# Gustavroot/DeflatedMLMC_Schwinger

Measured on AMD Instinct MI355X. Metric: hutchinson_probe_samples_per_sec_schwinger128, higher is better.
Workload: dtype f64

## Files before the change

### deflatedmlmc_schwinger_amd/csrc/sw_kernels.hpp

```cpp
#pragma once
#include <hip/hip_runtime.h>
#include <stdint.h>

namespace swk {

typedef double2 cplx;

#define SW_WAVE 64
#define SW_BLOCK 256
#define SW_WAVES_PER_BLOCK 4
#define SW_SHIFT_SMALL_L 256
#define SW_SHIFT_MID_L 768
#define SW_SHIFT_MAX_L 1024

__device__ __forceinline__ cplx cmake(double a, double b) { cplx r; r.x = a; r.y = b; return r; }
__device__ __forceinline__ cplx cadd(cplx a, cplx b) { return cmake(a.x + b.x, a.y + b.y); }
__device__ __forceinline__ cplx csub(cplx a, cplx b) { return cmake(a.x - b.x, a.y - b.y); }
__device__ __forceinline__ cplx cmul(cplx a, cplx b) {
  return cmake(fma(a.x, b.x, -a.y * b.y), fma(a.x, b.y, a.y * b.x));
}
__device__ __forceinline__ cplx cmulc(cplx a, cplx b) {
  return cmake(fma(a.x, b.x, a.y * b.y), fma(a.x, b.y, -a.y * b.x));
}
__device__ __forceinline__ void cfma(cplx& acc, cplx a, cplx b) {
// ... 585 lines not shown
  const int wave = threadIdx.x >> 6;
  const int lane = threadIdx.x & 63;
  const int bx = xcd_remap(blockIdx.x, gridDim.x);
  const int slot = __builtin_amdgcn_readfirstlane(bx * SW_WAVES_PER_BLOCK + wave);
  if (slot >= ngroups) return;
  const int grp = order ? __builtin_amdgcn_readfirstlane(order[slot]) : slot;
  const size_t col = (size_t)blockIdx.y * 64 + lane;
  const int* c = cols + (size_t)grp * K;
  const C* v = vals + (size_t)grp * K * G;
  C acc[G];
#pragma unroll
  for (int g = 0; g < G; ++g) acc[g] = czero<C>();
  const C* Xc = X + col;
  constexpr int UC = (G <= 8) ? 8 : 4;
  int k = 0;
  for (; k + UC <= K; k += UC) {
    C xs[UC];
#pragma unroll
    for (int u = 0; u < UC; ++u) xs[u] = Xc[(size_t)c[k + u] * nbp];
    __builtin_amdgcn_sched_barrier(0);
#pragma unroll
    for (int u = 0; u < UC; ++u) {
#pragma unroll
      for (int g = 0; g < G; ++g) cfma(acc[g], v[(size_t)(k + u) * G + g], xs[u]);
    }
  }
  for (; k < K; ++k) {
    const C x = Xc[(size_t)c[k] * nbp];
#pragma unroll
    for (int g = 0; g < G; ++g) cfma(acc[g], v[(size_t)k * G + g], x);
  }
#pragma unroll
  for (int g = 0; g < G; ++g) {
    const size_t row = (size_t)grp * G + g;
    C o = acc[g];
    if (MODE == 1) o = csub(B[row * nbp + col], o);
    if (MODE == 2) o = cadd(B[row * nbp + col], o);
    if (MODE == 3) {
      C t = X[row * nbp + col];
      cfma(t, w, csub(B[row * nbp + col], o));
      o = t;
    }
    Y[row * nbp + col] = o;
  }
}

typedef double sw_double4 __attribute__((ext_vector_type(4)));
#ifndef SW_BSR_WAVES_NT4
#define SW_BSR_WAVES_NT4 3
#endif
#define SW_BSR_MIN_WAVES(NT_, STG_) (((NT_) == 4 && (STG_) <= 4) ? SW_BSR_WAVES_NT4 : 1)

template <int MODE, int NT, bool NTIO>
__device__ __forceinline__ void bsr_store(const sw_double4 (&re)[NT], const sw_double4 (&im)[NT], int rt,
                                          int c0, int lane, const int* __restrict__ tmap,
                                          const double* __restrict__ Xr,
                                          const double* __restrict__ Br, double* __restrict__ Yr,
                                          int ld, cplx w, const double (*xown)[NT] = nullptr) {
  const int c = lane & 15;
  const bool odd = (c & 1) != 0;
  const int ot = tmap ? __builtin_amdgcn_readfirstlane(tmap[rt]) : rt;
#pragma unroll
  for (int r = 0; r < 4; ++r) {
    const size_t row = (size_t)ot * 16 + (lane >> 4) + 4 * r;
#pragma unroll
    for (int t = 0; t < NT; ++t) {
      const double s = __shfl_xor(im[t][r], 1);
      double y = odd ? re[t][r] + s : re[t][r] - s;
      const size_t off = row * ld + c0 + t * 16 + c;
      if (MODE == 1) y = (NTIO ? __builtin_nontemporal_load(&Br[off]) : Br[off]) - y;
      if (MODE == 3) {
        const double tt = (NTIO ? __builtin_nontemporal_load(&Br[off]) : Br[off]) - y;
        const double tp = __shfl_xor(tt, 1);
        y = (xown ? xown[r][t] : Xr[off]) + w.x * tt + (odd ? w.y * tp : -w.y * tp);
      }
      if (NTIO) __builtin_nontemporal_store(y, &Yr[off]);
      else Yr[off] = y;
    }
  }
}

template <int MODE, int NT, bool NTIO = false, int STG = 2>
__global__ __launch_bounds__(SW_BLOCK, SW_BSR_MIN_WAVES(NT, STG)) void k_bsr_mfma(const cplx* __restrict__ Ap,
                                                       const int* __restrict__ kcol, int KS,
                                                       int RT, const double* __restrict__ Xr,
                                                       const double* __restrict__ Br,
                                                       double* __restrict__ Yr, int ld, int nbp,
                                                       cplx w, int map, int msub,
                                                       const int* __restrict__ tmap, int xreg) {
  const int lane = threadIdx.x & 63;
  const int RB = (RT + SW_WAVES_PER_BLOCK - 1) / SW_WAVES_PER_BLOCK;
  const int NC = (gridDim.y > 1) ? gridDim.y : gridDim.x / RB;
  int bx, cy;
  if (gridDim.y > 1) {
    cy = blockIdx.y;
    bx = xcd_remap(blockIdx.x, RB);
  } else if (map == 0 || map == 3 || (RB & 7)) {
    cy = blockIdx.x / RB;
    bx = xcd_remap(blockIdx.x - cy * RB, RB);
  } else {
    const int xcd = blockIdx.x & 7, j = blockIdx.x >> 3, RBx = RB >> 3;
    if (map == 1 || (RBx % msub)) {
      cy = j % NC;
      bx = xcd * RBx + j / NC;
    } else {
      const int per = NC * msub;
      const int sidx = j / per, rem = j - sidx * per;
      cy = rem / msub;
      bx = xcd * RBx + sidx * msub + (rem - cy * msub);
    }
  }
  const int rt = __builtin_amdgcn_readfirstlane(bx * SW_WAVES_PER_BLOCK + (threadIdx.x >> 6));
  if (rt >= RT) return;
  const int c0 = cy * (16 * NT);
  const cplx* a = Ap + (size_t)rt * KS * 64 + lane;
  const int* kc = kcol + (size_t)rt * KS;
  const double* b = Xr + (size_t)(lane >> 4) * ld + c0 + (lane & 15);
  sw_double4 re[NT], im[NT];
#pragma unroll
  for (int t = 0; t < NT; ++t) {
    re[t] = sw_double4{0.0, 0.0, 0.0, 0.0};
    im[t] = re[t];
  }
#define SW_BSR_LOAD(M_, X_, KSI)                               \
  {                                                            \
    M_ = a[(size_t)(KSI) * 64];                                \
    const double* bk_ = b + (size_t)kc[(KSI)] * ld;            \
    _Pragma("unroll") for (int t = 0; t < NT; ++t) X_[t] = bk_[t * 16]; \
  }
#define SW_BSR_MFMA(M_, X_)                                                        \
  _Pragma("unroll") for (int t = 0; t < NT; ++t) {                                 \
    re[t] = __builtin_amdgcn_mfma_f64_16x16x4f64(M_.x, X_[t], re[t], 0, 0, 0);     \
    im[t] = __builtin_amdgcn_mfma_f64_16x16x4f64(M_.y, X_[t], im[t], 0, 0, 0);     \
  }
  cplx mm[STG];
  double xx[STG][NT];
#pragma unroll
  for (int s = 0; s < STG; ++s) SW_BSR_LOAD(mm[s], xx[s], s);
  for (int ks = 0; ks < KS; ks += STG) {
#pragma unroll
    for (int s = 0; s < STG; ++s) {
      const int kn = (ks + s + STG < KS) ? ks + s + STG : ks + s;
      __builtin_amdgcn_sched_barrier(0);
      SW_BSR_MFMA(mm[s], xx[s]);
      __builtin_amdgcn_sched_barrier(0);
      SW_BSR_LOAD(mm[s], xx[s], kn);
    }
  }
#undef SW_BSR_LOAD
#undef SW_BSR_MFMA
  if (MODE == 3 && STG == 4 && xreg) bsr_store<MODE, NT, NTIO>(re, im, rt, c0, lane, tmap, Xr, Br, Yr, ld, w, xx);
  else bsr_store<MODE, NT, NTIO>(re, im, rt, c0, lane, tmap, Xr, Br, Yr, ld, w);
}

#define SW_BSR3_MIN_WAVES(NT_, STG_) (((NT_) <= 2 && (STG_) <= 4) ? 2 : 1)

template <int MODE, int NT, bool NTIO = false, int STG = 4>
__global__ __launch_bounds__(SW_BLOCK, SW_BSR3_MIN_WAVES(NT, STG)) void k_bsr_mfma3(
    const cplx* __restrict__ Ap, const int* __restrict__ kcol, int KS, int RT, const cplx* __restrict__ X,
    const cplx* __restrict__ B, cplx* __restrict__ Y, int nbp, cplx w, int map, int msub,
    const int* __restrict__ tmap, int xreg) {
  const int lane = threadIdx.x & 63;
  const int RB = (RT + SW_WAVES_PER_BLOCK - 1) / SW_WAVES_PER_BLOCK;
  const int NC = gridDim.x / RB;
  int bx, cy;
  if (map == 0 || map == 3 || (RB & 7)) {
    cy = blockIdx.x / RB;
    bx = xcd_remap(blockIdx.x - cy * RB, RB);
  } else {
    const int xcd = blockIdx.x & 7, j = blockIdx.x >> 3, RBx = RB >> 3;
    if (map == 1 || (RBx % msub)) {
      cy = j % NC;
      bx = xcd * RBx + j / NC;
    } else {
      const int per = NC * msub;
      const int sidx = j / per, rem = j - sidx * per;
      cy = rem / msub;
      bx = xcd * RBx + sidx * msub + (rem - cy * msub);
    }
  }
  const int rt = __builtin_amdgcn_readfirstlane(bx * SW_WAVES_PER_BLOCK + (threadIdx.x >> 6));
  if (rt >= RT) return;
  const int c0 = cy * (16 * NT);
  const cplx* a = Ap + (size_t)rt * KS * 64 + lane;
  const int* kc = kcol + (size_t)rt * KS;
  const cplx* b = X + (size_t)(lane >> 4) * nbp + c0 + (lane & 15);
  sw_double4 t1[NT], t2[NT], t3[NT];
#pragma unroll
  for (int t = 0; t < NT; ++t) {
    t1[t] = sw_double4{0.0, 0.0, 0.0, 0.0};
    t2[t] = t1[t];
    t3[t] = t1[t];
  }
#define SW_B3_LOAD(M_, X_, KSI)                                 \
  {                                                             \
    M_ = a[(size_t)(KSI) * 64];                                 \
    const cplx* bk_ = b + (size_t)kc[(KSI)] * nbp;              \
    _Pragma("unroll") for (int t = 0; t < NT; ++t) X_[t] = bk_[t * 16]; \
  }
#define SW_B3_MFMA(M_, X_)                                                                  \
  {                                                                                         \
    const double ms_ = M_.x + M_.y;                                                         \
    _Pragma("unroll") for (int t = 0; t < NT; ++t) {                                        \
      t1[t] = __builtin_amdgcn_mfma_f64_16x16x4f64(M_.x, X_[t].x, t1[t], 0, 0, 0);          \
      t2[t] = __builtin_amdgcn_mfma_f64_16x16x4f64(M_.y, X_[t].y, t2[t], 0, 0, 0);          \
      t3[t] = __builtin_amdgcn_mfma_f64_16x16x4f64(ms_, X_[t].x + X_[t].y, t3[t], 0, 0, 0); \
    }                                                                                       \
  }
  cplx mm[STG];
  cplx xx[STG][NT];
#pragma unroll
  for (int s = 0; s < STG; ++s) SW_B3_LOAD(mm[s], xx[s], (s < KS ? s : 0));
  for (int ks = 0; ks < KS; ks += STG) {
#pragma unroll
    for (int s = 0; s < STG; ++s) {
      if (ks + s < KS) {
        const int kn = (ks + s + STG < KS) ? ks + s + STG : ks + s;
        __builtin_amdgcn_sched_barrier(0);
        SW_B3_MFMA(mm[s], xx[s]);
        __builtin_amdgcn_sched_barrier(0);
        SW_B3_LOAD(mm[s], xx[s], kn);
      }
    }
  }
#undef SW_B3_LOAD
#undef SW_B3_MFMA
  const int ot = tmap ? __builtin_amdgcn_readfirstlane(tmap[rt]) : rt;
  const bool own = MODE == 3 && STG == 4 && xreg && (KS % 4 == 0);
#pragma unroll
  for (int r = 0; r < 4; ++r) {
    const size_t row = (size_t)ot * 16 + (lane >> 4) + 4 * r;
#pragma unroll
    for (int t = 0; t < NT; ++t) {
      const size_t off = row * nbp + c0 + t * 16 + (lane & 15);
      cplx y = cmake(t1[t][r] - t2[t][r], t3[t][r] - t1[t][r] - t2[t][r]);
      if (MODE == 1 || MODE == 3) {
        cplx q;
        if (NTIO) {
          const double* bp_ = (const double*)&B[off];
          q = cmake(__builtin_nontemporal_load(bp_), __builtin_nontemporal_load(bp_ + 1));
        } else {
          q = B[off];
        }
        y = csub(q, y);
      }
      if (MODE == 3) {
        cplx o;
        if constexpr (STG == 4) o = own ? xx[r][t] : X[off];
        else o = X[off];
        cfma(o, w, y);
        y = o;
      }
      if (NTIO) {
        double* yp_ = (double*)&Y[off];
        __builtin_nontemporal_store(y.x, yp_);
        __builtin_nontemporal_store(y.y, yp_ + 1);
      } else {
        Y[off] = y;
      }
    }
  }
}

#define SW_DL_DEPTH 4

template <int RTW, int KB>
__global__ __launch_bounds__(128 * RTW) void k_dense_mfma3_lds(const cplx* __restrict__ Ap,
                                                              const int* __restrict__ kcol, int KS, int RT,
                                                              const cplx* __restrict__ X, cplx* __restrict__ Y,
                                                              int nbp, const int* __restrict__ tmap) {
  constexpr int WAVES = 2 * RTW;
  constexpr int APIECES = RTW * KB, PIECES = APIECES + 2 * KB, PPW = PIECES / WAVES;
  static_assert(PIECES % WAVES == 0, "pieces must divide over the waves");
  __shared__ cplx lds[2][PIECES * 64];
  const int lane = threadIdx.x & 63;
  const int wave = __builtin_amdgcn_readfirstlane((int)(threadIdx.x >> 6));
  const int RB = RT / RTW, NC = nbp >> 5;
  int rb, pc;
  if ((RB & 7) == 0) {
    const int xcd = blockIdx.x & 7, j = blockIdx.x >> 3, RBx = RB >> 3;
    rb = xcd * RBx + j / NC;
    pc = j % NC;
  } else {
    rb = blockIdx.x / NC;
    pc = blockIdx.x % NC;
  }
  const int rtl = wave >> 1, ptl = wave & 1;
  const int rt0 = rb * RTW;
  const int c0 = pc * 32;
  const int nstages = KS / KB;
  static_assert(APIECES % WAVES == 0 && PPW >= 3 && PPW <= 6, "piece layout");
#define SW_DL_SRC(T)                                                                                     \
  ((WAVES * (T) < APIECES)                                                                               \
       ? Ap + ((size_t)(rt0 + (wave + WAVES * (T)) / KB) * KS + ((wave + WAVES * (T)) % KB)) * 64 + lane \
       : X + (size_t)(2 * ((wave + WAVES * (T) - APIECES) & 1) + (lane >> 5)) * nbp + c0 + (lane & 31))
  const cplx* const src0 = SW_DL_SRC(0);
  const cplx* const src1 = SW_DL_SRC(1);
  const cplx* const src2 = SW_DL_SRC(2);
  const cplx* const src3 = (PPW > 3) ? SW_DL_SRC(3) : src2;
  const cplx* const src4 = (PPW > 4) ? SW_DL_SRC(4) : src2;
  const cplx* const src5 = (PPW > 5) ? SW_DL_SRC(5) : src2;
#undef SW_DL_SRC
#define SW_DL_XK(T) ((wave + WAVES * (T) - APIECES) >> 1)
#define SW_DL_LD1(DST, SRC, T, KS0)                                                                \
  if (WAVES * (T) < APIECES) DST = SRC[(size_t)(KS0) * 64];                                        \
  else DST = SRC[(size_t)kcol[(KS0) + SW_DL_XK(T)] * nbp];
#define SW_DL_LOAD(RING, ST)                                                                       \
  {                                                                                                \
    const int ks0_ = min((ST), nstages - 1) * KB;                                                  \
    SW_DL_LD1(RING##_0, src0, 0, ks0_)                                                             \
    SW_DL_LD1(RING##_1, src1, 1, ks0_)                                                             \
    SW_DL_LD1(RING##_2, src2, 2, ks0_)                                                             \
    if (PPW > 3) { SW_DL_LD1(RING##_3, src3, 3, ks0_) }                                            \
    if (PPW > 4) { SW_DL_LD1(RING##_4, src4, 4, ks0_) }                                            \
    if (PPW > 5) { SW_DL_LD1(RING##_5, src5, 5, ks0_) }                                            \
  }
#define SW_DL_WRITE(RING, BUF)                                                                     \
  {                                                                                                \
    lds[BUF][(wave + WAVES * 0) * 64 + lane] = RING##_0;                                           \
    lds[BUF][(wave + WAVES * 1) * 64 + lane] = RING##_1;                                           \
    lds[BUF][(wave + WAVES * 2) * 64 + lane] = RING##_2;                                           \
    if (PPW > 3) lds[BUF][(wave + WAVES * 3) * 64 + lane] = RING##_3;                              \
    if (PPW > 4) lds[BUF][(wave + WAVES * 4) * 64 + lane] = RING##_4;                              \
    if (PPW > 5) lds[BUF][(wave + WAVES * 5) * 64 + lane] = RING##_5;                              \
  }
#define SW_DL_DECL(RING) \
  cplx RING##_0, RING##_1, RING##_2, RING##_3 = cmake(0.0, 0.0), RING##_4 = RING##_3, RING##_5 = RING##_3;
  SW_DL_DECL(ring0)
  SW_DL_DECL(ring1)
  SW_DL_DECL(ring2)
  SW_DL_DECL(ring3)
#undef SW_DL_DECL
  static_assert(SW_DL_DEPTH == 4, "the ring is written out for four stages");
#define SW_DL_STEP(RING, BUF, ST)                                                                  \
  {                                                                                                \
    SW_DL_WRITE(RING, (BUF) ^ 1);                                                                  \
    __builtin_amdgcn_sched_barrier(0);                                                             \
    SW_DL_LOAD(RING, (ST) + 1 + SW_DL_DEPTH);                                                      \
    __builtin_amdgcn_sched_barrier(0);                                                             \
    const cplx* sl_ = &lds[BUF][0];                                                                \
    _Pragma("unroll") for (int k = 0; k < KB; ++k) {                                               \
      const cplx m_ = sl_[a_off + k * 64];                                                         \
      const cplx xv_ = sl_[x_off + k * 128];                                                       \
      t1 = __builtin_amdgcn_mfma_f64_16x16x4f64(m_.x, xv_.x, t1, 0, 0, 0);                         \
      t2 = __builtin_amdgcn_mfma_f64_16x16x4f64(m_.y, xv_.y, t2, 0, 0, 0);                         \
      t3 = __builtin_amdgcn_mfma_f64_16x16x4f64(m_.x + m_.y, xv_.x + xv_.y, t3, 0, 0, 0);          \
    }                                                                                              \
    __syncthreads();                                                                               \
  }
  SW_DL_LOAD(ring0, 0);
  SW_DL_LOAD(ring1, 1);
  SW_DL_LOAD(ring2, 2);
  SW_DL_LOAD(ring3, 3);
  SW_DL_WRITE(ring0, 0);
  __builtin_amdgcn_sched_barrier(0);
  SW_DL_LOAD(ring0, 4);
  __builtin_amdgcn_sched_barrier(0);
  __syncthreads();
  sw_double4 t1 = {0.0, 0.0, 0.0, 0.0}, t2 = t1, t3 = t1;
  const int a_off = (rtl * KB) * 64 + lane;
  const int x_off = (APIECES + (lane >> 5)) * 64 + ((lane >> 4) & 1) * 32 + ptl * 16 + (lane & 15);
  for (int st = 0; st < nstages; st += 4) {
    SW_DL_STEP(ring1, 0, st);
    SW_DL_STEP(ring2, 1, st + 1);
    SW_DL_STEP(ring3, 0, st + 2);
    SW_DL_STEP(ring0, 1, st + 3);
  }
#undef SW_DL_STEP
#undef SW_DL_LOAD
#undef SW_DL_LD1
#undef SW_DL_XK
#undef SW_DL_WRITE
  const int rt = rt0 + rtl;
  const int ot = tmap ? __builtin_amdgcn_readfirstlane(tmap[rt]) : rt;
#pragma unroll
  for (int r = 0; r < 4; ++r) {
    const size_t row = (size_t)ot * 16 + (lane >> 4) + 4 * r;
    Y[row * nbp + c0 + ptl * 16 + (lane & 15)] = cmake(t1[r] - t2[r], t3[r] - t1[r] - t2[r]);
  }
}

typedef float sw_float4 __attribute__((ext_vector_type(4)));

template <int MODE, int NT, int STG>
__global__ __launch_bounds__(SW_BLOCK) void k_bsr_mfma_f32(const cplxf* __restrict__ Ap,
                                                           const int* __restrict__ kcol, int KS,
                                                           int RT, const cplxf* __restrict__ X,
                                                           const cplxf* __restrict__ B,
                                                           cplxf* __restrict__ Y, int nbp, cplxf w,
                                                           int map, const int* __restrict__ tmap) {
  const int lane = threadIdx.x & 63;
  const int RB = (RT + SW_WAVES_PER_BLOCK - 1) / SW_WAVES_PER_BLOCK;
  const int NC = gridDim.x / RB;
  int bx, cy;
  if (map == 0 || (RB & 7)) {
    cy = blockIdx.x / RB;
    bx = xcd_remap(blockIdx.x - cy * RB, RB);
  } else {
    const int xcd = blockIdx.x & 7, j = blockIdx.x >> 3, RBx = RB >> 3;
    cy = j % NC;
    bx = xcd * RBx + j / NC;
  }
  const int rt = __builtin_amdgcn_readfirstlane(bx * SW_WAVES_PER_BLOCK + (threadIdx.x >> 6));
  if (rt >= RT) return;
  const int c0 = cy * (16 * NT);
  const cplxf* a = Ap + (size_t)rt * KS * 64 + lane;
  const int* kc = kcol + (size_t)rt * KS;
  const cplxf* b = X + (size_t)(lane >> 4) * nbp + c0 + (lane & 15);
  sw_float4 re[NT], im[NT];
#pragma unroll
  for (int t = 0; t < NT; ++t) {
    re[t] = sw_float4{0.f, 0.f, 0.f, 0.f};
    im[t] = re[t];
  }
#define SW_BSRF_LOAD(M_, X_, KSI)                               \
  {                                                             \
    M_ = a[(size_t)(KSI) * 64];                                 \
    const cplxf* bk_ = b + (size_t)kc[(KSI)] * nbp;             \
    _Pragma("unroll") for (int t = 0; t < NT; ++t) X_[t] = bk_[t * 16]; \
  }
#define SW_BSRF_MFMA(M_, X_)                                                              \
  {                                                                                       \
    const float nay_ = -M_.y;                                                             \
    _Pragma("unroll") for (int t = 0; t < NT; ++t) {                                      \
      re[t] = __builtin_amdgcn_mfma_f32_16x16x4f32(M_.x, X_[t].x, re[t], 0, 0, 0);        \
      im[t] = __builtin_amdgcn_mfma_f32_16x16x4f32(M_.x, X_[t].y, im[t], 0, 0, 0);        \
    }                                                                                     \
    _Pragma("unroll") for (int t = 0; t < NT; ++t) {                                      \
      re[t] = __builtin_amdgcn_mfma_f32_16x16x4f32(nay_, X_[t].y, re[t], 0, 0, 0);        \
      im[t] = __builtin_amdgcn_mfma_f32_16x16x4f32(M_.y, X_[t].x, im[t], 0, 0, 0);        \
    }                                                                                     \
  }
  cplxf mm[STG];
  cplxf xx[STG][NT];
#pragma unroll
  for (int s = 0; s < STG; ++s) SW_BSRF_LOAD(mm[s], xx[s], (s < KS ? s : 0));
  for (int ks = 0; ks < KS; ks += STG) {
#pragma unroll
    for (int s = 0; s < STG; ++s) {
      if (ks + s < KS) {
        const int kn = (ks + s + STG < KS) ? ks + s + STG : ks + s;
        __builtin_amdgcn_sched_barrier(0);
        SW_BSRF_MFMA(mm[s], xx[s]);
        __builtin_amdgcn_sched_barrier(0);
        SW_BSRF_LOAD(mm[s], xx[s], kn);
      }
    }
  }
#undef SW_BSRF_LOAD
#undef SW_BSRF_MFMA
  const int ot = tmap ? __builtin_amdgcn_readfirstlane(tmap[rt]) : rt;
#pragma unroll
  for (int r = 0; r < 4; ++r) {
    const size_t row = (size_t)ot * 16 + 4 * (lane >> 4) + r;
#pragma unroll
    for (int t = 0; t < NT; ++t) {
      const size_t off = row * nbp + c0 + t * 16 + (lane & 15);
      cplxf y = cmake(re[t][r], im[t][r]);
      if (MODE == 1) y = csub(B[off], y);
      if (MODE == 3) {
        cplxf o = X[off];
        cfma(o, w, csub(B[off], y));
        y = o;
      }
      Y[off] = y;
    }
  }
}

template <int MODE, int NT>
__global__ __launch_bounds__(SW_BLOCK) void k_bsr_mfma_f32_sk(const cplxf* __restrict__ Ap,
                                                              const int* __restrict__ kcol, int KS,
                                                              int RT, const cplxf* __restrict__ X,
                                                              const cplxf* __restrict__ B,
                                                              cplxf* __restrict__ Y, int nbp, cplxf w,
                                                              const int* __restrict__ tmap) {
  __shared__ float red[3][NT * 8][64];
  const int lane = threadIdx.x & 63;
  const int q = threadIdx.x >> 6;
  const int rt = blockIdx.x % RT;
  const int cy = blockIdx.x / RT;
  const int c0 = cy * (16 * NT);
  const cplxf* a = Ap + (size_t)rt * KS * 64 + lane;
  const int* kc = kcol + (size_t)rt * KS;
  const cplxf* b = X + (size_t)(lane >> 4) * nbp + c0 + (lane & 15);
  sw_float4 re[NT], im[NT];
#pragma unroll
  for (int t = 0; t < NT; ++t) {
    re[t] = sw_float4{0.f, 0.f, 0.f, 0.f};
    im[t] = re[t];
  }
  constexpr int STG = 4;
  cplxf mm[STG];
  cplxf xx[STG][NT];
#define SW_SKF_LOAD(S_, KSI)                                                  \
  {                                                                           \
    const int ks_ = ((KSI) < KS) ? (KSI) : q;                                 \
    mm[S_] = a[(size_t)ks_ * 64];                                             \
    const cplxf* bk_ = b + (size_t)kc[ks_] * nbp;                             \
    _Pragma("unroll") for (int t = 0; t < NT; ++t) xx[S_][t] = bk_[t * 16];   \
  }
#pragma unroll
  for (int s = 0; s < STG; ++s) SW_SKF_LOAD(s, q + 4 * s);
  for (int ks = q; ks < KS; ks += 4 * STG) {
#pragma unroll
    for (int s = 0; s < STG; ++s) {
      if (ks + 4 * s < KS) {
        __builtin_amdgcn_sched_barrier(0);
        const float nay = -mm[s].y;
#pragma unroll
        for (int t = 0; t < NT; ++t) {
          re[t] = __builtin_amdgcn_mfma_f32_16x16x4f32(mm[s].x, xx[s][t].x, re[t], 0, 0, 0);
          im[t] = __builtin_amdgcn_mfma_f32_16x16x4f32(mm[s].x, xx[s][t].y, im[t], 0, 0, 0);
        }
#pragma unroll
        for (int t = 0; t < NT; ++t) {
          re[t] = __builtin_amdgcn_mfma_f32_16x16x4f32(nay, xx[s][t].y, re[t], 0, 0, 0);
          im[t] = __builtin_amdgcn_mfma_f32_16x16x4f32(mm[s].y, xx[s][t].x, im[t], 0, 0, 0);
        }
        __builtin_amdgcn_sched_barrier(0);
        SW_SKF_LOAD(s, ks + 4 * s + 4 * STG);
      }
    }
  }
#undef SW_SKF_LOAD
  if (q > 0) {
#pragma unroll
    for (int t = 0; t < NT; ++t)
#pragma unroll
      for (int r = 0; r < 4; ++r) {
        red[q - 1][t * 8 + r][lane] = re[t][r];
        red[q - 1][t * 8 + 4 + r][lane] = im[t][r];
      }
  }
  __syncthreads();
  if (q != 0) return;
  const int ot = tmap ? __builtin_amdgcn_readfirstlane(tmap[rt]) : rt;
#pragma unroll
  for (int r = 0; r < 4; ++r) {
    const size_t row = (size_t)ot * 16 + 4 * (lane >> 4) + r;
#pragma unroll
    for (int t = 0; t < NT; ++t) {
      const size_t off = row * nbp + c0 + t * 16 + (lane & 15);
      cplxf y = cmake(re[t][r] + red[0][t * 8 + r][lane] + red[1][t * 8 + r][lane] + red[2][t * 8 + r][lane],
                      im[t][r] + red[0][t * 8 + 4 + r][lane] + red[1][t * 8 + 4 + r][lane] +
                          red[2][t * 8 + 4 + r][lane]);
      if (MODE == 1) y = csub(B[off], y);
      if (MODE == 3) {
        cplxf o = X[off];
        cfma(o, w, csub(B[off], y));
        y = o;
      }
      Y[off] = y;
    }
  }
}

template <class CI, class CO>
__global__ __launch_bounds__(SW_BLOCK) void k_cast(const CI* __restrict__ src, CO* __restrict__ dst,
                                                   size_t count) {
  const size_t i = (size_t)blockIdx.x * SW_BLOCK + threadIdx.x;
  if (i >= count) return;
  const CI v = src[i];
  CO o;
  o.x = (typename real_of<CO>::type)v.x;
  o.y = (typename real_of<CO>::type)v.y;
  dst[i] = o;
}

__device__ __forceinline__ int blk_pos_row(int q) { return q & 15; }
__device__ __forceinline__ int blk_pos_col(int q) { return 4 * (q >> 6) + ((q & 63) >> 4); }

__global__ __launch_bounds__(256) void k_block_inverse(const cplx* __restrict__ src,
                                                       const long long* __restrict__ soff,
                                                       cplx* __restrict__ dst,
                                                       const long long* __restrict__ doff,
                                                       int* __restrict__ info) {
  __shared__ cplx a[16][33];
  __shared__ cplx fac[16];
  __shared__ int piv;
  const int q = threadIdx.x;
  const int i = blk_pos_row(q), c = blk_pos_col(q);
  const cplx* s = src + soff[blockIdx.x];
  a[i][c] = s[q];
  a[i][16 + c] = cmake(i == c ? 1.0 : 0.0, 0.0);
  __syncthreads();
  for (int k = 0; k < 16; ++k) {
    if (q == 0) {
      int p = k;
      double best = a[k][k].x * a[k][k].x + a[k][k].y * a[k][k].y;
      for (int r = k + 1; r < 16; ++r) {
        const double m = a[r][k].x * a[r][k].x + a[r][k].y * a[r][k].y;
        if (m > best) {
          best = m;
          p = r;
        }
      }
      piv = p;
      if (best == 0.0) atomicOr(info, 1);
    }
    __syncthreads();
    const int p = piv;
    if (p != k && q < 32) {
      const cplx t = a[k][q];
      a[k][q] = a[p][q];
      a[p][q] = t;
    }
    __syncthreads();
    if (q < 16) fac[q] = a[q][k];
    __syncthreads();
    const cplx pv = fac[k];
    const double d = pv.x * pv.x + pv.y * pv.y;
    const cplx ip = d > 0.0 ? cmake(pv.x / d, -pv.y / d) : cmake(0.0, 0.0);
    if (q < 32) a[k][q] = cmul(a[k][q], ip);
    __syncthreads();
#pragma unroll
    for (int e = 0; e < 2; ++e) {
      const int idx = q + 256 * e;
      const int r = idx >> 5, cc = idx & 31;
      if (r != k) {
        const cplx f = fac[r];
        const cplx t = cmul(f, a[k][cc]);
        a[r][cc] = csub(a[r][cc], t);
      }
    }
    __syncthreads();
  }
  dst[doff[blockIdx.x] + q] = a[i][16 + c];
}

__global__ __launch_bounds__(256) void k_block_products(const int* __restrict__ ptr,
                                                        const long long* __restrict__ aoff,
                                                        const long long* __restrict__ boff,
                                                        const cplx* __restrict__ A,
                                                        const cplx* __restrict__ B,
                                                        const long long* __restrict__ ioff,
                                                        const cplx* __restrict__ init, double sign,
                                                        cplx* __restrict__ out,
                                                        const long long* __restrict__ ooff) {
  __shared__ cplx as[16][17], bs[16][17];
  const int q = threadIdx.x;
  const int i = blk_pos_row(q), c = blk_pos_col(q);
  const int b = blockIdx.x;
  cplx acc = cmake(0.0, 0.0);
  for (int t = ptr[b]; t < ptr[b + 1]; ++t) {
    as[i][c] = A[aoff[t] + q];
    bs[i][c] = B[boff[t] + q];
    __syncthreads();
#pragma unroll
    for (int m = 0; m < 16; ++m) cfma(acc, as[i][m], bs[m][c]);
    __syncthreads();
  }
  cplx o = cmake(sign * acc.x, sign * acc.y);
  if (ioff[b] >= 0) o = cadd(o, init[ioff[b] + q]);
  out[ooff[b] + q] = o;
}

__global__ __launch_bounds__(1024) void k_gj_pivot(const cplx* __restrict__ A, int n, int k,
                                                   int* __restrict__ pivs, cplx* __restrict__ pvinv,
                                                   int* __restrict__ info) {
  __shared__ double bm[1024];
  __shared__ int bi[1024];
  const int t = threadIdx.x;
  double best = -1.0;
  int arg = k;
  for (int r = k + t; r < n; r += 1024) {
    const cplx v = A[(size_t)r * n + k];
    const double m = v.x * v.x + v.y * v.y;
    if (m > best) {
      best = m;
      arg = r;
    }
  }
// ... 2788 lines not shown
```

Before: 35060.

## Software-pipeline LDS reads and MFMAs, prefetch kcol indices a stage early

Restructures the inner f64 MFMA loop of the BSR dot kernel so that LDS operand reads for the next k-step, and the complex-sum adds, are interleaved with the MFMAs of the current step. The last MFMA triple of each stage is deferred into the next stage to overlap with its ring write and global load issue. It also loads the kcol column indices into registers one stage ahead, taking the dependent index load off the X gather path. The cost is more live registers and a more intricate schedule held in place by sched_barriers.

Measured after the change: 35260 (median of 4 runs). No clear change (+0.6%).

```diff
diff --git a/deflatedmlmc_schwinger_amd/csrc/sw_kernels.hpp b/deflatedmlmc_schwinger_amd/csrc/sw_kernels.hpp
--- a/deflatedmlmc_schwinger_amd/csrc/sw_kernels.hpp
+++ b/deflatedmlmc_schwinger_amd/csrc/sw_kernels.hpp
@@ -911,9 +911,18 @@
   const cplx* const src5 = (PPW > 5) ? SW_DL_SRC(5) : src2;
 #undef SW_DL_SRC
 #define SW_DL_XK(T) ((wave + WAVES * (T) - APIECES) >> 1)
+  int kc_0 = 0, kc_1 = 0, kc_2 = 0, kc_3 = 0, kc_4 = 0, kc_5 = 0;
+#define SW_DL_KC1(T, KS0) \
+  if ((T) < PPW && WAVES * (T) >= APIECES) kc_##T = kcol[(KS0) + SW_DL_XK(T)];
+#define SW_DL_KC(ST)                                                                               \
+  {                                                                                                \
+    const int kk0_ = min((ST), nstages - 1) * KB;                                                  \
+    SW_DL_KC1(0, kk0_) SW_DL_KC1(1, kk0_) SW_DL_KC1(2, kk0_)                                       \
+    SW_DL_KC1(3, kk0_) SW_DL_KC1(4, kk0_) SW_DL_KC1(5, kk0_)                                       \
+  }
 #define SW_DL_LD1(DST, SRC, T, KS0)                                                                \
   if (WAVES * (T) < APIECES) DST = SRC[(size_t)(KS0) * 64];                                        \
-  else DST = SRC[(size_t)kcol[(KS0) + SW_DL_XK(T)] * nbp];
+  else DST = SRC[(size_t)kc_##T * nbp];
 #define SW_DL_LOAD(RING, ST)                                                                       \
   {                                                                                                \
     const int ks0_ = min((ST), nstages - 1) * KB;                                                  \
@@ -941,32 +950,68 @@
   SW_DL_DECL(ring3)
 #undef SW_DL_DECL
   static_assert(SW_DL_DEPTH == 4, "the ring is written out for four stages");
+  static_assert(KB % 2 == 0, "the k-steps of a stage alternate between two operand sets");
+#define SW_DL_READ(S, BUF, K)                                                                      \
+  {                                                                                                \
+    m##S = lds[BUF][a_off + (K) * 64];                                                             \
+    x##S = lds[BUF][x_off + (K) * 128];                                                            \
+  }
+#define SW_DL_SUMS(S)                                                                              \
+  {                                                                                                \
+    ms##S = m##S.x + m##S.y;                                                                       \
+    xs##S = x##S.x + x##S.y;                                                                       \
+  }
+#define SW_DL_MFMA(S)                                                                              \
+  {                                                                                                \
+    t1 = __builtin_amdgcn_mfma_f64_16x16x4f64(m##S.x, x##S.x, t1, 0, 0, 0);                        \
+    t2 = __builtin_amdgcn_mfma_f64_16x16x4f64(m##S.y, x##S.y, t2, 0, 0, 0);                        \
+    t3 = __builtin_amdgcn_mfma_f64_16x16x4f64(ms##S, xs##S, t3, 0, 0, 0);                          \
+  }
 #define SW_DL_STEP(RING, BUF, ST)                                                                  \
   {                                                                                                \
+    SW_DL_READ(P, BUF, 0);                                                                         \
+    __builtin_amdgcn_sched_barrier(0);                                                             \
+    SW_DL_MFMA(Q);                                                                                 \
+    __builtin_amdgcn_sched_barrier(0);                                                             \
     SW_DL_WRITE(RING, (BUF) ^ 1);                                                                  \
     __builtin_amdgcn_sched_barrier(0);                                                             \
     SW_DL_LOAD(RING, (ST) + 1 + SW_DL_DEPTH);                                                      \
     __builtin_amdgcn_sched_barrier(0);                                                             \
-    const cplx* sl_ = &lds[BUF][0];                                                                \
-    _Pragma("unroll") for (int k = 0; k < KB; ++k) {                                               \
-      const cplx m_ = sl_[a_off + k * 64];                                                         \
-      const cplx xv_ = sl_[x_off + k * 128];                                                       \
-      t1 = __builtin_amdgcn_mfma_f64_16x16x4f64(m_.x, xv_.x, t1, 0, 0, 0);                         \
-      t2 = __builtin_amdgcn_mfma_f64_16x16x4f64(m_.y, xv_.y, t2, 0, 0, 0);                         \
-      t3 = __builtin_amdgcn_mfma_f64_16x16x4f64(m_.x + m_.y, xv_.x + xv_.y, t3, 0, 0, 0);          \
+    _Pragma("unroll") for (int k = 0; k < KB; k += 2) {                                            \
+      SW_DL_SUMS(P);                                                                               \
+      __builtin_amdgcn_sched_barrier(0);                                                           \
+      SW_DL_READ(Q, BUF, k + 1);                                                                   \
+      if (k == KB - 2) SW_DL_KC((ST) + 2 + SW_DL_DEPTH);                                           \
+      __builtin_amdgcn_sched_barrier(0);                                                           \
+      SW_DL_MFMA(P);                                                                               \
+      SW_DL_SUMS(Q);                                                                               \
+      __builtin_amdgcn_sched_barrier(0);                                                           \
+      if (k + 2 < KB) {                                                                            \
+        SW_DL_READ(P, BUF, k + 2);                                                                 \
+        __builtin_amdgcn_sched_barrier(0);                                                         \
+        SW_DL_MFMA(Q);                                                                             \
+      }                                                                                            \
     }                                                                                              \
     __syncthreads();                                                                               \
   }
+  SW_DL_KC(0);
   SW_DL_LOAD(ring0, 0);
+  SW_DL_KC(1);
   SW_DL_LOAD(ring1, 1);
+  SW_DL_KC(2);
   SW_DL_LOAD(ring2, 2);
+  SW_DL_KC(3);
   SW_DL_LOAD(ring3, 3);
+  SW_DL_KC(4);
   SW_DL_WRITE(ring0, 0);
   __builtin_amdgcn_sched_barrier(0);
   SW_DL_LOAD(ring0, 4);
+  SW_DL_KC(1 + SW_DL_DEPTH);
   __builtin_amdgcn_sched_barrier(0);
   __syncthreads();
   sw_double4 t1 = {0.0, 0.0, 0.0, 0.0}, t2 = t1, t3 = t1;
+  cplx mP, xP, mQ = cmake(0.0, 0.0), xQ = mQ;
+  double msP, xsP, msQ = 0.0, xsQ = 0.0;
   const int a_off = (rtl * KB) * 64 + lane;
   const int x_off = (APIECES + (lane >> 5)) * 64 + ((lane >> 4) & 1) * 32 + ptl * 16 + (lane & 15);
   for (int st = 0; st < nstages; st += 4) {
@@ -975,9 +1020,15 @@
     SW_DL_STEP(ring3, 0, st + 2);
     SW_DL_STEP(ring0, 1, st + 3);
   }
+  SW_DL_MFMA(Q);
 #undef SW_DL_STEP
+#undef SW_DL_READ
+#undef SW_DL_SUMS
+#undef SW_DL_MFMA
 #undef SW_DL_LOAD
 #undef SW_DL_LD1
+#undef SW_DL_KC
+#undef SW_DL_KC1
 #undef SW_DL_XK
 #undef SW_DL_WRITE
   const int rt = rt0 + rtl;
```
